# dkales/dpf-go

Hardware: AMD Instinct MI355X
Metric: DPF leaf points/sec (EvalFull logN=20, batched keys) + AES blocks/sec (higher is better)
Workload: dtype u32

## Files before the change

dpf-go_amd/csrc/dpf_capi.hip:

```cpp
#include <hip/hip_runtime.h>
#include <sched.h>
#include <stdint.h>
#include <stdio.h>
#include <stdlib.h>
#include <string.h>
#include <sys/mman.h>

#include <algorithm>
#include <atomic>
#include <condition_variable>
#include <functional>
#include <memory>
#include <mutex>
#include <unordered_map>
#include <string>
#include <thread>
#include <vector>

#include "../../include/dpf_hip.h"
#include "dpf_internal.hpp"
#include "bs_kernels.hpp"
#include "dpf_kernels.hpp"
#include "pir_kernels.hpp"

// ... 324 lines not shown
}

bool want_bs() { return g_aes_impl.load(std::memory_order_relaxed) == DPF_AES_BITSLICED; }

hipError_t expand_keys(const uint8_t* d_keys, size_t klen, size_t nk, uint32_t stop, const TreeWs& w, hipStream_t st,
                       bool bs) {
    if (bs) return dpfk::launch_unpack_both(d_keys, klen, nk, stop, w.ek, w.ekb, st);
    return dpfk::launch_unpack(d_keys, klen, nk, stop, w.ek, st);
}

hipError_t run_tree(const TreeWs& w, size_t k0, size_t n, uint32_t stop, uint32_t prefix_bits, uint64_t prefix,
                    uint8_t* out, uint64_t stride, hipStream_t st, bool bs) {
    if (bs && dpfk::bs_applicable(stop, prefix_bits))
        return dpfk::launch_evalfull_bs(w.ek + k0 * dpfk::ek_words(stop), w.ekb + k0 * dpfk::bs_key_words(stop), n, stop,
                                        prefix_bits, prefix, out, stride, w.frontier, st);
    return dpfk::launch_evalfull(w.ek + k0 * dpfk::ek_words(stop), n, stop, prefix_bits, prefix, out, stride, st);
}

hipError_t tree_from_keys(const uint8_t* d_keys, size_t klen, size_t nk, uint32_t stop, uint32_t prefix_bits,
                          uint64_t prefix, uint8_t* out, uint64_t stride, void* d_work, hipStream_t st, bool bs,
                          bool* expanded) {
    if (!bs && dpfk::evalfull_raw_ok(nk, stop, prefix_bits)) {
        *expanded = false;
        return dpfk::launch_evalfull_raw(d_keys, klen, nk, stop, prefix_bits, prefix, out, stride, st);
    }
    *expanded = true;
    const TreeWs w = tree_ws(d_work, nk, stop);
    hipError_t e = expand_keys(d_keys, klen, nk, stop, w, st, bs);
    return e != hipSuccess ? e : run_tree(w, 0, nk, stop, prefix_bits, prefix, out, stride, st, bs);
}

constexpr size_t kStageBytes = (size_t)32 << 20;
constexpr size_t kSlabMinOut = (size_t)8 << 20;

int ensure_staging(Dev& d, size_t chunk_cap) {
    if (!d.cst) {
        HIP_TRY(hipStreamCreateWithFlags(&d.cst, hipStreamNonBlocking));
        for (int i = 0; i < 2; ++i) {
            HIP_TRY(hipEventCreateWithFlags(&d.ev_k[i], hipEventDisableTiming));
// ... 61 lines not shown
    HIP_TRY(hipMemcpyAsync(d.keys.p, keys, nk * klen, hipMemcpyHostToDevice, d.st));
    const TreeWs w = tree_ws(d.work.p, nk, stop);
    const bool bs = want_bs();
    const uint8_t* dk = (const uint8_t*)d.keys.p;
    uint32_t pb = 0;
    while ((olen >> pb) > kStageBytes) ++pb;
    if (olen >= kSlabMinOut && pb < 2) pb = 2;
    const bool raw = !bs && (pb == 0 ? dpfk::evalfull_raw_ok(std::min(per, nk), stop, 0) &&
                                                       (nk % per == 0 || dpfk::evalfull_raw_ok(nk % per, stop, 0))
                                                 : dpfk::evalfull_raw_ok(1, stop, pb));
    if (!raw) HIP_TRY(expand_keys(dk, klen, nk, stop, w, d.st, bs));
    if (pb == 0) {
        const size_t nch = (nk + per - 1) / per;
        return pipeline_d2h(d, nch, std::min(per, nk) * olen, [&](size_t i, uint8_t* dbuf, size_t& bytes, size_t& off) {
            const size_t k0 = i * per, n = std::min(per, nk - k0);
            if (raw) HIP_TRY(dpfk::launch_evalfull_raw(dk + k0 * klen, klen, n, stop, 0, 0, dbuf, olen, d.st));
            else HIP_TRY(run_tree(w, k0, n, stop, 0, 0, dbuf, olen, d.st, bs));
            bytes = n * olen;
            off = k0 * olen;
            return DPF_OK;
        }, out, nk * olen);
    }
    const size_t slab = olen >> pb, per_key = (size_t)1 << pb;
    return pipeline_d2h(d, nk * per_key, slab, [&](size_t i, uint8_t* dbuf, size_t& bytes, size_t& off) {
        const size_t k = i / per_key, p = i % per_key;
        if (raw) HIP_TRY(dpfk::launch_evalfull_raw(dk + k * klen, klen, 1, stop, pb, p, dbuf, slab, d.st));
        else HIP_TRY(run_tree(w, k, 1, stop, pb, p, dbuf, slab, d.st, bs));
        bytes = slab;
        off = k * olen + p * slab;
        return DPF_OK;
    }, out, nk * olen);
}

size_t pir_ek_bytes(size_t nkeys, uint32_t logN);
size_t eval_work_bytes(size_t nkeys, size_t ppk, uint32_t logN);

int eval_on_device(Dev& d, const uint8_t* keys, size_t klen, size_t nk, const uint64_t* xs, size_t ppk,
                   uint32_t logN, uint8_t* out) {
    std::lock_guard<std::mutex> lk(d.mu);
    DeviceGuard g(d.id);
    const uint32_t stop = stop_of(logN);
// ... 298 lines not shown
        std::lock_guard<std::mutex> lk(d.mu);
        DeviceGuard gd(d.id);
        HIP_TRY(hipError_t(d.keys.ensure(klen)));
        HIP_TRY(hipError_t(d.work.ensure(tree_ws_bytes(1, stop, pb, 1))));
        HIP_TRY(hipMemcpyAsync(d.keys.p, key, klen, hipMemcpyHostToDevice, d.st));
        const TreeWs w = tree_ws(d.work.p, 1, stop);
        const bool bs = want_bs();
        const uint8_t* dk = (const uint8_t*)d.keys.p;
        uint32_t extra = 0;
        while ((slab >> extra) > kStageBytes && pb + extra < stop) ++extra;
        const size_t sub = slab >> extra;
        const bool raw = !bs && dpfk::evalfull_raw_ok(1, stop, pb + extra);
        if (!raw) HIP_TRY(expand_keys(dk, klen, 1, stop, w, d.st, bs));
        return pipeline_d2h(d, (size_t)1 << extra, sub, [&](size_t j, uint8_t* dbuf, size_t& bytes, size_t& off) {
            const uint64_t p = ((uint64_t)lo << extra) + j;
            if (raw) HIP_TRY(dpfk::launch_evalfull_raw(dk, klen, 1, stop, pb + extra, p, dbuf, sub, d.st));
            else HIP_TRY(run_tree(w, 0, 1, stop, pb + extra, p, dbuf, sub, d.st, bs));
            bytes = sub;
            off = lo * slab + j * sub;
            return DPF_OK;
        }, out + lo * slab, slab, lo * slab);
    });
}

int dpf_evalfull_subtree_dev(int device, const uint8_t* d_keys, size_t klen, size_t nkeys, uint32_t logN,
                             uint32_t prefix_bits, uint64_t prefix, uint8_t* d_out, void* d_work, void* stream) {
    if (int rc = check_key(klen, logN)) return rc;
    const uint32_t stop = stop_of(logN);
    if (prefix_bits > stop || (prefix_bits < 64 && (prefix >> prefix_bits) != 0))
        return fail(DPF_ERR_PARAM, "dpf: subtree prefix out of range");
    if (nkeys == 0) return DPF_OK;
    DeviceGuard g(device);
    CuScope cus(stream);
    const bool bs = want_bs();
    bool expanded = false;
    forget_expanded(d_work);
    HIP_TRY(tree_from_keys(d_keys, klen, nkeys, stop, prefix_bits, prefix, d_out, (uint64_t)16 << (stop - prefix_bits),
                           d_work, (hipStream_t)stream, bs, &expanded));
    if (expanded) note_expanded(d_work, nkeys, stop, bs);
    return DPF_OK;
}

int dpf_evalfull_batch_dev(int device, const uint8_t* d_keys, size_t klen, size_t nkeys, uint32_t logN,
                           uint8_t* d_out, void* d_work, void* stream) {
    return dpf_evalfull_subtree_dev(device, d_keys, klen, nkeys, logN, 0, 0, d_out, d_work, stream);
}

size_t dpf_eval_workspace_size(size_t nkeys, size_t pts_per_key, uint32_t logN) {
    return std::max<size_t>(16, eval_work_bytes(nkeys, pts_per_key, logN));
}

uint32_t dpf_eval_frontier_level(uint32_t logN, size_t pts_per_key) {
    return logN > 63 ? 0 : dpfk::eval_frontier_level(stop_of(logN), pts_per_key);
}
// ... 417 lines not shown
```

dpf-go_amd/csrc/dpf_kernels.hip:

```cpp
#include <hip/hip_runtime.h>
#include <stdint.h>
#include <stdlib.h>

#include <algorithm>
#include <atomic>
#include <cmath>
#include <mutex>
#include <type_traits>
#include "aes_consts.hpp"
#include "aes_ttable.hpp"
#include "dpf_kernels.hpp"
#include "wave_prio.hpp"
#include "tree_ops.hpp"

namespace dpfk {

#ifdef DPF_WAVE_TIMES
constexpr uint64_t kWaveTimesMax = 1u << 16;
__device__ uint64_t g_wave_times[5 * kWaveTimesMax];
#endif

struct Ctx {
    const uint8_t* tab;
    uint32_t lo;
    KeySrc ks;
    Blk fcw;
    uint8_t* outp;
    uint4* nseed;
    uint8_t* nt;
    uint32_t groups;
    uint32_t* prog = nullptr;
    uint32_t pslot = 0;
};

// ... 55 lines not shown
        ob = leaf_fix(ob, b.t, c.fcw);
        o2 = oa;
        o3 = ob;
        if (h == 0) {
            o0 = oa;
            o1 = ob;
        }
        m = pend;
    }
    store16(p, o0);
    store16(p + 16, o1);
    store16(p + 32, o2);
    store16(p + 48, o3);
}

template <int DMAX, int D, bool NODES, bool PAIR, bool B, bool RAW = false>
__device__ __forceinline__ void dfs(Ctx& c, uint32_t lvl0, const Node& n) {
    if constexpr (PAIR && D == 3) {
        CW cw = key_cw<RAW>(c.ks, lvl0 + DMAX - 3);
        Node L, R;
        expand<B>(c.tab, c.lo, n, cw, L, R);
        const bool odd = (threadIdx.x & 1u) != 0;
        const Node got = pair_swap(sel(odd, L, R));
        const int64_t sub = 16ll << DMAX;
        Node cur = sel(odd, got, L);
        const Node second = sel(odd, R, got);
#pragma nounroll
        for (int h = 0; h < 2; ++h) {
            leaves4<B, RAW>(c, lvl0 + DMAX - 2, cur, c.outp + (h == 0 ? (odd ? 64 - sub : 0) : (odd ? 64 : sub)));
            prio_step<DMAX>(c);
            cur = second;
        }
        c.outp += 128;
    } else if constexpr (D == 0) {
        if constexpr (NODES) {
            emit_node(c, n);
        } else {
            Blk o = mmo1(c.tab, c.lo, KeyFixed<false>{}, n.s);
            store16(c.outp, leaf_fix(o, n.t, c.fcw));
            c.outp += 16;
        }
    } else if constexpr (D == 2 && !NODES) {
        leaves4<B, RAW>(c, lvl0 + DMAX - 2, n, c.outp);
// ... 24 lines not shown
        } else {
            Blk oL, oR;
            mmo2<B>(c.tab, c.lo, KeyFixed<false>{}, L.s, oL, KeyFixed<false>{}, R.s, oR);
            store16(c.outp, leaf_fix(oL, L.t, c.fcw));
            store16(c.outp + 16, leaf_fix(oR, R.t, c.fcw));
            c.outp += 32;
        }
    } else {
        CW cw = key_cw<RAW>(c.ks, lvl0 + DMAX - D);
        Node L, R;
        expand<B>(c.tab, c.lo, n, cw, L, R);
        Node ch = L;
        const Node pend = R;
#pragma nounroll
        for (int side = 0; side < 2; ++side) {
            dfs<DMAX, D - 1, NODES, PAIR, B, RAW>(c, lvl0, ch);
            ch = pend;
        }
    }
}

__global__ void k_unpack(const uint8_t* __restrict__ keys, uint64_t key_len, uint64_t nkeys, uint32_t stop,
                         uint32_t* __restrict__ ek) {
    const uint64_t recs = (uint64_t)stop + 2;
    const uint64_t i = (uint64_t)blockIdx.x * blockDim.x + threadIdx.x;
    if (i >= nkeys * recs) return;
    const uint64_t k = i / recs, r = i % recs;
    const uint8_t* kp = keys + k * key_len;
    uint32_t* o = ek + k * (recs * 8) + r * 8;
    auto w = [](const uint8_t* p) {
        return (uint32_t)p[0] | ((uint32_t)p[1] << 8) | ((uint32_t)p[2] << 16) | ((uint32_t)p[3] << 24);
    };
    if (r == 0) {
        o[0] = w(kp); o[1] = w(kp + 4); o[2] = w(kp + 8); o[3] = w(kp + 12);
        o[4] = kp[16]; o[5] = 0; o[6] = 0; o[7] = 0;
    } else if (r <= stop) {
        const uint8_t* p = kp + 17 + 18 * (r - 1);
        o[0] = w(p); o[1] = w(p + 4); o[2] = w(p + 8); o[3] = w(p + 12);
        o[4] = p[16]; o[5] = p[17]; o[6] = 0; o[7] = 0;
    } else {
        const uint8_t* p = kp + key_len - 16;
        o[0] = w(p); o[1] = w(p + 4); o[2] = w(p + 8); o[3] = w(p + 12);
        o[4] = 0; o[5] = 0; o[6] = 0; o[7] = 0;
    }
}

template <int D, bool UNIFORM, bool NODES, bool RAW = false>
__global__ __launch_bounds__(kTreeBlockMax, kTreeWaves) void k_evalfull(const uint32_t* __restrict__ ekeys, uint32_t stop,
                                                        uint64_t nunits, uint32_t units_log, uint32_t ltop,
                                                        uint64_t sub_base, uint8_t* __restrict__ out,
                                                        uint8_t* __restrict__ out_t, uint64_t out_stride,
                                                        uint64_t klen = 0, uint64_t kboff = 0) {
    static_assert(!RAW || (UNIFORM && !NODES), "raw keys: wave-uniform leaf launches only");
#ifdef DPF_WAVE_TIMES
    const uint64_t t_start = wall_clock64();
#endif
    __shared__ __attribute__((aligned(16))) uint32_t s_tab[kTabWords];
    const uint32_t B = blockDim.x, W = 31u - (uint32_t)__builtin_clz(B);
    const uint64_t u = (uint64_t)blockIdx.x * B + threadIdx.x;
    uint64_t key = u >> units_log;
    if constexpr (UNIFORM) key = __builtin_amdgcn_readfirstlane((uint32_t)key);
    const uint64_t local = u & ((1ull << units_log) - 1);
    const uint64_t sub = sub_base + local;
    Ctx c;
    if constexpr (RAW) {
        c.ks = {nullptr, ekeys, kboff + key * klen, klen};
    } else {
        c.ks = {ekeys + key * ((uint64_t)(stop + 2) * 8), nullptr, 0, 0};
// ... 80 lines not shown
            n = get(threadIdx.x >> (W - F));
            lvl = l1;
        }
    }
    if (cw_lds) {
        for (uint32_t i = lvl; i < ltop; ++i)
            walk_step<true>(c.tab, c.lo, n, lds_cw(i), (uint32_t)(sub >> (ltop - 1 - i)) & 1u);
    } else {
        for (uint32_t i = lvl; i < ltop; ++i)
            walk_step<true>(c.tab, c.lo, n, key_cw<RAW>(c.ks, i), (uint32_t)(sub >> (ltop - 1 - i)) & 1u);
    }
#ifdef DPF_WAVE_TIMES
    const uint64_t t_walk = wall_clock64();
#endif
    constexpr bool kPair = UNIFORM && !NODES && D >= 3;
    dfs<D, D, NODES, kPair, UNIFORM, RAW>(c, ltop, n);
    if (c.prog != nullptr) c.prog[c.pslot] = 0xffffffffu;
#ifdef DPF_WAVE_TIMES
    if ((threadIdx.x & 63) == 0) {
        const uint64_t wv = u >> 6;
        if (wv < kWaveTimesMax) {
            g_wave_times[5 * wv] = t_start;
            g_wave_times[5 * wv + 1] = wall_clock64();
            g_wave_times[5 * wv + 2] = __builtin_amdgcn_s_getreg(0xF804);
            g_wave_times[5 * wv + 3] = __builtin_amdgcn_s_getreg(0xF814);
            g_wave_times[5 * wv + 4] = t_walk;
        }
    }
#endif
}

__device__ __forceinline__ Node eval_start(const uint32_t* ek, uint64_t key, uint64_t x, uint32_t logN,
                                           const uint4* fseed, const uint8_t* ft, uint32_t L) {
    Node n;
    if (fseed != nullptr) {
        const uint64_t idx = (key << L) + ((x >> (logN - L)) & ((1ull << L) - 1));
        const uint4 v = fseed[idx];
        n.s = {v.x, v.y, v.z, v.w};
        n.t = ft[idx];
    } else {
        n.s = load_blk(ek);
// ... 437 lines not shown
    while (b < maxb && n > cus * b) b <<= 1;
    return b;
}

struct TreeShape {
    uint32_t d, block;
};
static TreeShape pick_shape(uint32_t span, uint64_t nkeys, bool nodes, uint32_t prefix_bits) {
    static const int forced = [] {
        const char* e = getenv("DPF_SUBTREE_DEPTH");
        return e ? atoi(e) : -1;
    }();
    const uint32_t dmax = span < kMaxD ? span : kMaxD;
    auto threads = [&](uint32_t dd) { return span - dd >= 40 ? ~0ull : nkeys << (span - dd); };
    auto block = [&](uint32_t dd) {
        return pick_block(threads(dd), !nodes && dd >= kBigMinD ? (uint32_t)kTreeBlockBig : (uint32_t)kTreeBlock);
    };
    if (forced >= 0) {
        const uint32_t d = dmax < (uint32_t)forced ? dmax : (uint32_t)forced;
        return {d, block(d)};
    }
    constexpr double kLat = 1.9e-6;
    constexpr double kPerWave = 0.2e-6;
    const double wave_slots = 64.0 * cu_count();
    uint32_t best = dmax;
    double best_t = 1e30;
    for (int dd = (int)dmax; dd >= 0; --dd) {
        const uint32_t d = (uint32_t)dd;
        double walk = (double)(span - d), lat = 0.0;
        const double w = (double)threads(d) / wave_slots;
        const double rounds = w > 16.0 ? std::ceil(w / 16.0) : 1.0;
// ... 34 lines not shown
}
template <class F>
static void with_depth(uint32_t d, F&& f) {
    switch (d) {
        case 0: return f(std::integral_constant<int, 0>{});
        case 1: return f(std::integral_constant<int, 1>{});
        case 2: return f(std::integral_constant<int, 2>{});
        case 3: return f(std::integral_constant<int, 3>{});
        case 4: return f(std::integral_constant<int, 4>{});
        case 5: return f(std::integral_constant<int, 5>{});
        case 6: return f(std::integral_constant<int, 6>{});
        default: return f(std::integral_constant<int, 7>{});
    }
}

template <bool NODES>
static hipError_t launch_tree(const uint32_t* ek, uint64_t nkeys, uint32_t stop, uint32_t depth,
                              uint32_t prefix_bits, uint64_t prefix, uint8_t* out, uint8_t* out_t,
                              uint64_t out_stride, hipStream_t st) {
    const TreeLaunch t = tree_launch(nkeys, depth, prefix_bits, prefix, NODES);
    if (t.nunits == 0) return hipSuccess;
    with_depth(t.d, [&](auto dd) {
        constexpr int D = decltype(dd)::value;
        if (t.units_log >= 6)
            hipLaunchKernelGGL((k_evalfull<D, true, NODES>), t.grid, t.block, 0, st, ek, stop, t.nunits, t.units_log,
                               t.ltop, t.sub_base, out, out_t, out_stride);
        else
            hipLaunchKernelGGL((k_evalfull<D, false, NODES>), t.grid, t.block, 0, st, ek, stop, t.nunits, t.units_log,
                               t.ltop, t.sub_base, out, out_t, out_stride);
    });
    return hipGetLastError();
}

bool evalfull_raw_ok(uint64_t nkeys, uint32_t stop, uint32_t prefix_bits) {
    static const bool on = [] {
        const char* e = getenv("DPF_RAW_KEYS");
        return !(e && e[0] == '0');
    }();
    if (!on || nkeys == 0 || prefix_bits > stop) return false;
    return tree_launch(nkeys, stop, prefix_bits, 0, false).units_log >= 6;
}

hipError_t launch_evalfull_raw(const uint8_t* keys, uint64_t klen, uint64_t nkeys, uint32_t stop, uint32_t prefix_bits,
                               uint64_t prefix, uint8_t* out, uint64_t out_stride, hipStream_t st) {
    const TreeLaunch t = tree_launch(nkeys, stop, prefix_bits, prefix, false);
    if (t.units_log < 6) return hipErrorInvalidValue;
    const uint64_t kboff = (uintptr_t)keys & 3;
    const uint32_t* kw = reinterpret_cast<const uint32_t*>(keys - kboff);
    with_depth(t.d, [&](auto dd) {
        hipLaunchKernelGGL((k_evalfull<decltype(dd)::value, true, false, true>), t.grid, t.block, 0, st, kw, stop,
                           t.nunits, t.units_log, t.ltop, t.sub_base, out, nullptr, out_stride, klen, kboff);
    });
    return hipGetLastError();
}

hipError_t launch_nodes(const uint32_t* ek, uint64_t nkeys, uint32_t stop, uint32_t depth, uint32_t prefix_bits,
                        uint64_t prefix, uint8_t* seeds, uint8_t* ts, uint64_t stride, hipStream_t st) {
    return launch_tree<true>(ek, nkeys, stop, depth, prefix_bits, prefix, seeds, ts, stride, st);
}

hipError_t launch_evalfull(const uint32_t* ek, uint64_t nkeys, uint32_t stop, uint32_t prefix_bits,
                           uint64_t prefix, uint8_t* out, uint64_t out_stride, hipStream_t st) {
    return launch_tree<false>(ek, nkeys, stop, stop, prefix_bits, prefix, out, nullptr, out_stride, st);
}

uint32_t eval_frontier_level(uint32_t stop, uint64_t pts_per_key) {
    uint32_t L = 0;
    while (L < kMaxFrontierHbm && L < stop && (2ull << (L + 1)) <= pts_per_key) ++L;
    static const int shift = [] {
        const char* e = getenv("DPF_EVAL_LEVEL_SHIFT");
        return e && *e ? atoi(e) : 0;
    }();
    if (L >= 4 && shift > 0 && L + (uint32_t)shift < stop && L + (uint32_t)shift <= kMaxFrontierHbm) L += shift;
    return L >= 4 ? L : 0;
}

uint64_t eval_frontier_bytes(uint64_t nkeys, uint32_t stop, uint64_t pts_per_key) {
    const uint32_t L = eval_frontier_level(stop, pts_per_key);
// ... 95 lines not shown
```

dpf-go_amd/csrc/dpf_kernels.hpp:

```cpp
#pragma once
#include <hip/hip_runtime.h>
#include <stdint.h>

namespace dpfk {

constexpr int kBlock = 512;
constexpr int kTreeBlock = 512;
constexpr int kTreeBlockBig = 1024;
constexpr int kTreeBlockMax = 1024;
constexpr uint32_t kBigMinD = 6;
constexpr uint32_t kFeedbackMinD = 6;
constexpr int kTreeWaves = 4;
constexpr uint32_t kMaxD = 7;
constexpr uint32_t kMaxFrontierHbm = 16;

void set_cu_budget(int cus);
int cu_budget();
int cu_count();

inline uint64_t ek_words(uint32_t stop) { return ((uint64_t)stop + 2) * 8; }

hipError_t launch_mmo_tt(const uint8_t* in, uint8_t* out, uint64_t nblocks, uint32_t right, uint32_t reps,
                         hipStream_t st);

hipError_t launch_unpack(const uint8_t* keys, uint64_t key_len, uint64_t nkeys, uint32_t stop, uint32_t* ek,
                         hipStream_t st);

hipError_t launch_evalfull(const uint32_t* ek, uint64_t nkeys, uint32_t stop, uint32_t prefix_bits,
                           uint64_t prefix, uint8_t* out, uint64_t out_stride, hipStream_t st);

bool evalfull_raw_ok(uint64_t nkeys, uint32_t stop, uint32_t prefix_bits);
hipError_t launch_evalfull_raw(const uint8_t* keys, uint64_t klen, uint64_t nkeys, uint32_t stop, uint32_t prefix_bits,
                               uint64_t prefix, uint8_t* out, uint64_t out_stride, hipStream_t st);

hipError_t launch_nodes(const uint32_t* ek, uint64_t nkeys, uint32_t stop, uint32_t depth, uint32_t prefix_bits,
                        uint64_t prefix, uint8_t* seeds, uint8_t* ts, uint64_t stride, hipStream_t st);

uint32_t eval_frontier_level(uint32_t stop, uint64_t pts_per_key);
int set_eval_trie(int on);
int get_eval_trie();
bool eval_trie_built();
uint64_t eval_frontier_bytes(uint64_t nkeys, uint32_t stop, uint64_t pts_per_key);
hipError_t launch_eval(const uint32_t* ek, uint32_t stop, uint32_t logN, const uint64_t* xs, uint64_t nq,
                       uint64_t pts_per_key, uint8_t* out, void* frontier, uint64_t frontier_bytes,
                       hipStream_t st);

}
```

dpf-go_amd/dpf/__init__.py:

```python
from __future__ import annotations

import ctypes
import os
from typing import Optional, Sequence, Tuple

import numpy as np

_HERE = os.path.dirname(os.path.abspath(__file__))
LIB_PATH = os.environ.get("DPF_LIB") or os.path.join(os.path.dirname(_HERE), "lib", "libdpf_hip.so")
HEADER_PATH = os.path.join(os.path.dirname(os.path.dirname(_HERE)), "include", "dpf_hip.h")

DPF_OK = 0
DPF_ERR_PARAM = -1
DPF_ERR_KEYLEN = -2
DPF_ERR_NODEV = -3
DPF_ERR_HIP = -4
DPF_ERR_NOMEM = -5
AES_TTABLE = 0
AES_BITSLICED = 1


class DPFPanic(RuntimeError):

    def __init__(self, code: int, msg: str):
# ... 18 lines not shown
    "dpf_gpu_init_devices": (_int, [ctypes.POINTER(_int), _int]),
    "dpf_gpu_shutdown": (None, []),
    "dpf_gpu_count": (_int, []),
    "dpf_gen_seeded": (_int, [_u64, _u32, _u8p, _u8p, _u8p, _u8p]),
    "dpf_gen": (_int, [_u64, _u32, _u8p, _u8p]),
    "dpf_gen_batch_seeded": (_int, [_u64p, _u32, _u8p, _u8p, _sz, _u8p, _u8p, _int]),
    "dpf_keys_pack": (_int, [ctypes.POINTER(_vp), ctypes.POINTER(_sz), _sz, _sz, _u8p]),
    "dpf_keys_unpack": (_int, [_u8p, _sz, _sz, ctypes.POINTER(_vp)]),
    "dpf_eval": (_int, [_u8p, _sz, _u64, _u32, _u8p]),
    "dpf_evalfull": (_int, [_u8p, _sz, _u32, _u8p]),
    "dpf_evalfull_batch": (_int, [_u8p, _sz, _sz, _u32, _u8p, _int]),
    "dpf_eval_batch": (_int, [_u8p, _sz, _sz, _u64p, _sz, _u32, _u8p, _int]),
    "dpf_evalfull_split": (_int, [_u8p, _sz, _u32, _u8p, _int]),
    "dpf_evalfull_batch_dev": (_int, [_int, _vp, _sz, _sz, _u32, _vp, _vp, _vp]),
    "dpf_evalfull_subtree_dev": (_int, [_int, _vp, _sz, _sz, _u32, _u32, _u64, _vp, _vp, _vp]),
    "dpf_eval_workspace_size": (_sz, [_sz, _sz, _u32]),
    "dpf_eval_frontier_level": (_u32, [_u32, _sz]),
    "dpf_eval_batch_dev": (_int, [_int, _vp, _sz, _sz, _vp, _sz, _u32, _vp, _vp, _sz, _vp]),
    "dpf_expand_keys_dev": (_int, [_int, _vp, _sz, _sz, _u32, _vp, _vp]),
    "dpf_evalfull_expanded_dev": (_int, [_int, _vp, _sz, _u32, _u32, _u64, _vp, _vp]),
    "dpf_forget_workspace": (_int, [_vp]),
    "dpf_set_small_call_path": (_int, [_int]),
    "dpf_get_small_call_path": (_int, []),
    "dpf_small_call_max_logN": (ctypes.c_uint32, []),
    "dpf_set_aes_impl": (_int, [_int]),
    "dpf_get_aes_impl": (_int, []),
    "dpf_set_eval_kernel": (_int, [_int]),
    "dpf_get_eval_kernel": (_int, []),
    "dpf_set_pir_kernel": (_int, [_int]),
    "dpf_get_pir_kernel": (_int, []),
# ... 59 lines not shown
    return np.frombuffer(bytes(b), dtype=np.uint8)


def key_len(logN: int) -> int:
    return int(lib().dpf_key_len(logN))


def evalfull_len(logN: int) -> int:
    return int(lib().dpf_evalfull_len(logN))


def workspace_size(nkeys: int, logN: int) -> int:
    return int(lib().dpf_workspace_size(nkeys, logN))


def gpu_init(ngpus: int = 0) -> int:
    rc = lib().dpf_gpu_init(ngpus)
    if rc < 0:
        _check(rc)
    return rc


def gpu_init_devices(ordinals: Sequence[int]) -> int:
    ids = (_int * len(ordinals))(*ordinals)
    rc = lib().dpf_gpu_init_devices(ids, len(ordinals))
    if rc < 0:
        _check(rc)
    return rc


# ... 371 lines not shown
```

include/dpf_hip.h:

```cpp
#ifndef DPF_HIP_H
#define DPF_HIP_H

#include <stddef.h>
#include <stdint.h>

#ifdef __cplusplus
extern "C" {
#endif

#define DPF_OK 0
#define DPF_ERR_PARAM (-1)
#define DPF_ERR_KEYLEN (-2)
#define DPF_ERR_NODEV (-3)
#define DPF_ERR_HIP (-4)
#define DPF_ERR_NOMEM (-5)

const char* dpf_last_error(void);

size_t dpf_key_len(uint32_t logN);
size_t dpf_evalfull_len(uint32_t logN);
size_t dpf_workspace_size(size_t nkeys, uint32_t logN);

int dpf_gpu_init(int ngpus);
int dpf_gpu_init_devices(const int* ordinals, int n);
// ... 6 lines not shown
int dpf_gen_batch_seeded(const uint64_t* alphas, uint32_t logN, const uint8_t* s0s, const uint8_t* s1s, size_t n,
                         uint8_t* kas, uint8_t* kbs, int nthreads);

int dpf_keys_pack(const uint8_t* const* keys, const size_t* lens, size_t n, size_t key_len, uint8_t* out);
int dpf_keys_unpack(const uint8_t* packed, size_t key_len, size_t n, uint8_t* const* keys);

int dpf_eval(const uint8_t* key, size_t key_len, uint64_t x, uint32_t logN, uint8_t* out_bit);
int dpf_evalfull(const uint8_t* key, size_t key_len, uint32_t logN, uint8_t* out);
int dpf_evalfull_batch(const uint8_t* keys, size_t key_len, size_t nkeys, uint32_t logN, uint8_t* out, int ngpus);
int dpf_eval_batch(const uint8_t* keys, size_t key_len, size_t nkeys, const uint64_t* xs, size_t pts_per_key,
                   uint32_t logN, uint8_t* out, int ngpus);
int dpf_evalfull_split(const uint8_t* key, size_t key_len, uint32_t logN, uint8_t* out, int ngpus);

int dpf_evalfull_batch_dev(int device, const uint8_t* d_keys, size_t key_len, size_t nkeys, uint32_t logN,
                           uint8_t* d_out, void* d_work, void* stream);
int dpf_evalfull_subtree_dev(int device, const uint8_t* d_keys, size_t key_len, size_t nkeys, uint32_t logN,
                             uint32_t prefix_bits, uint64_t prefix, uint8_t* d_out, void* d_work, void* stream);
size_t dpf_eval_workspace_size(size_t nkeys, size_t pts_per_key, uint32_t logN);
uint32_t dpf_eval_frontier_level(uint32_t logN, size_t pts_per_key);
int dpf_eval_batch_dev(int device, const uint8_t* d_keys, size_t key_len, size_t nkeys, const uint64_t* d_xs,
                       size_t pts_per_key, uint32_t logN, uint8_t* d_out, void* d_work, size_t work_bytes,
                       void* stream);

int dpf_stream_create_cu_masked(int device, uint32_t cu_first, uint32_t cu_count, void** stream);
int dpf_stream_destroy(void* stream);

#define DPF_AES_TTABLE 0
#define DPF_AES_BITSLICED 1
int dpf_set_aes_impl(int impl);
int dpf_get_aes_impl(void);
// ... 70 lines not shown
```

Measured before the change: 4618 billion.

## Add inter-wave work stealing for deep EvalFull leaf subtrees and tune block choice

Adds an optional work-stealing scheme to the tree evaluation kernel. Each wave expands its subtree frontier into a shared workspace and publishes progress. Idle waves scan for unfinished jobs and claim trailing units through atomics, to even out tail imbalance. Stealing is off by default behind an environment variable. The launch heuristic is also changed to choose between big and small blocks by comparing idle CUs against extra blocks, which can change occupancy for mid-sized launches.

```diff
diff --git a/dpf-go_amd/csrc/dpf_capi.hip b/dpf-go_amd/csrc/dpf_capi.hip
--- a/dpf-go_amd/csrc/dpf_capi.hip
+++ b/dpf-go_amd/csrc/dpf_capi.hip
@@ -362,7 +362,8 @@
     if (bs && dpfk::bs_applicable(stop, prefix_bits))
         return dpfk::launch_evalfull_bs(w.ek + k0 * dpfk::ek_words(stop), w.ekb + k0 * dpfk::bs_key_words(stop), n, stop,
                                         prefix_bits, prefix, out, stride, w.frontier, st);
-    return dpfk::launch_evalfull(w.ek + k0 * dpfk::ek_words(stop), n, stop, prefix_bits, prefix, out, stride, st);
+    return dpfk::launch_evalfull(w.ek + k0 * dpfk::ek_words(stop), n, stop, prefix_bits, prefix, out, stride, st,
+                                 w.frontier);
 }
 
 hipError_t tree_from_keys(const uint8_t* d_keys, size_t klen, size_t nk, uint32_t stop, uint32_t prefix_bits,
@@ -370,7 +371,8 @@
                           bool* expanded) {
     if (!bs && dpfk::evalfull_raw_ok(nk, stop, prefix_bits)) {
         *expanded = false;
-        return dpfk::launch_evalfull_raw(d_keys, klen, nk, stop, prefix_bits, prefix, out, stride, st);
+        return dpfk::launch_evalfull_raw(d_keys, klen, nk, stop, prefix_bits, prefix, out, stride, st,
+                                         d_work != nullptr ? tree_ws(d_work, nk, stop).frontier : nullptr);
     }
     *expanded = true;
     const TreeWs w = tree_ws(d_work, nk, stop);
@@ -462,7 +464,7 @@
         const size_t nch = (nk + per - 1) / per;
         return pipeline_d2h(d, nch, std::min(per, nk) * olen, [&](size_t i, uint8_t* dbuf, size_t& bytes, size_t& off) {
             const size_t k0 = i * per, n = std::min(per, nk - k0);
-            if (raw) HIP_TRY(dpfk::launch_evalfull_raw(dk + k0 * klen, klen, n, stop, 0, 0, dbuf, olen, d.st));
+            if (raw) HIP_TRY(dpfk::launch_evalfull_raw(dk + k0 * klen, klen, n, stop, 0, 0, dbuf, olen, d.st, w.frontier));
             else HIP_TRY(run_tree(w, k0, n, stop, 0, 0, dbuf, olen, d.st, bs));
             bytes = n * olen;
             off = k0 * olen;
@@ -472,7 +474,7 @@
     const size_t slab = olen >> pb, per_key = (size_t)1 << pb;
     return pipeline_d2h(d, nk * per_key, slab, [&](size_t i, uint8_t* dbuf, size_t& bytes, size_t& off) {
         const size_t k = i / per_key, p = i % per_key;
-        if (raw) HIP_TRY(dpfk::launch_evalfull_raw(dk + k * klen, klen, 1, stop, pb, p, dbuf, slab, d.st));
+        if (raw) HIP_TRY(dpfk::launch_evalfull_raw(dk + k * klen, klen, 1, stop, pb, p, dbuf, slab, d.st, w.frontier));
         else HIP_TRY(run_tree(w, k, 1, stop, pb, p, dbuf, slab, d.st, bs));
         bytes = slab;
         off = k * olen + p * slab;
@@ -801,7 +803,7 @@
         if (!raw) HIP_TRY(expand_keys(dk, klen, 1, stop, w, d.st, bs));
         return pipeline_d2h(d, (size_t)1 << extra, sub, [&](size_t j, uint8_t* dbuf, size_t& bytes, size_t& off) {
             const uint64_t p = ((uint64_t)lo << extra) + j;
-            if (raw) HIP_TRY(dpfk::launch_evalfull_raw(dk, klen, 1, stop, pb + extra, p, dbuf, sub, d.st));
+            if (raw) HIP_TRY(dpfk::launch_evalfull_raw(dk, klen, 1, stop, pb + extra, p, dbuf, sub, d.st, w.frontier));
             else HIP_TRY(run_tree(w, 0, 1, stop, pb + extra, p, dbuf, sub, d.st, bs));
             bytes = sub;
             off = lo * slab + j * sub;
@@ -825,6 +827,13 @@
     HIP_TRY(tree_from_keys(d_keys, klen, nkeys, stop, prefix_bits, prefix, d_out, (uint64_t)16 << (stop - prefix_bits),
                            d_work, (hipStream_t)stream, bs, &expanded));
     if (expanded) note_expanded(d_work, nkeys, stop, bs);
+    return DPF_OK;
+}
+
+int dpf_tree_steal_stats(int device, uint64_t* stolen, uint64_t* run_twice) {
+    if (stolen == nullptr || run_twice == nullptr) return fail(DPF_ERR_PARAM, "dpf: null statistics pointer");
+    DeviceGuard g(device);
+    HIP_TRY(dpfk::steal_last_stats(stolen, run_twice));
     return DPF_OK;
 }
 
diff --git a/dpf-go_amd/csrc/dpf_kernels.hip b/dpf-go_amd/csrc/dpf_kernels.hip
--- a/dpf-go_amd/csrc/dpf_kernels.hip
+++ b/dpf-go_amd/csrc/dpf_kernels.hip
@@ -7,17 +7,20 @@
 #include <cmath>
 #include <mutex>
 #include <type_traits>
+#include <vector>
 #include "aes_consts.hpp"
 #include "aes_ttable.hpp"
 #include "dpf_kernels.hpp"
 #include "wave_prio.hpp"
 #include "tree_ops.hpp"
+#include "tree_steal.hpp"
 
 namespace dpfk {
 
 #ifdef DPF_WAVE_TIMES
 constexpr uint64_t kWaveTimesMax = 1u << 16;
-__device__ uint64_t g_wave_times[5 * kWaveTimesMax];
+constexpr int kWaveTimesCols = 7;
+__device__ uint64_t g_wave_times[kWaveTimesCols * kWaveTimesMax];
 #endif
 
 struct Ctx {
@@ -103,19 +106,23 @@
     store16(p + 48, o3);
 }
 
-template <int DMAX, int D, bool NODES, bool PAIR, bool B, bool RAW = false>
-__device__ __forceinline__ void dfs(Ctx& c, uint32_t lvl0, const Node& n) {
+struct NoHook {
+    __device__ __forceinline__ void operator()() const {}
+};
+template <int DMAX, int D, bool NODES, bool PAIR, bool B, bool RAW = false, int SUBLOG = DMAX, class Hook = NoHook>
+__device__ __forceinline__ void dfs(Ctx& c, uint32_t lvl0, const Node& n, const Hook& hook = Hook{}) {
     if constexpr (PAIR && D == 3) {
         CW cw = key_cw<RAW>(c.ks, lvl0 + DMAX - 3);
         Node L, R;
         expand<B>(c.tab, c.lo, n, cw, L, R);
         const bool odd = (threadIdx.x & 1u) != 0;
         const Node got = pair_swap(sel(odd, L, R));
-        const int64_t sub = 16ll << DMAX;
+        const int64_t sub = 16ll << SUBLOG;
         Node cur = sel(odd, got, L);
         const Node second = sel(odd, R, got);
 #pragma nounroll
         for (int h = 0; h < 2; ++h) {
+            if (h == 1) hook();
             leaves4<B, RAW>(c, lvl0 + DMAX - 2, cur, c.outp + (h == 0 ? (odd ? 64 - sub : 0) : (odd ? 64 : sub)));
             prio_step<DMAX>(c);
             cur = second;
@@ -170,10 +177,171 @@
         const Node pend = R;
 #pragma nounroll
         for (int side = 0; side < 2; ++side) {
-            dfs<DMAX, D - 1, NODES, PAIR, B, RAW>(c, lvl0, ch);
+            dfs<DMAX, D - 1, NODES, PAIR, B, RAW, SUBLOG>(c, lvl0, ch);
             ch = pend;
         }
     }
+}
+
+struct StealOps {
+    static __device__ __forceinline__ uint32_t load(const uint32_t& w) {
+        return __hip_atomic_load(&w, __ATOMIC_RELAXED, __HIP_MEMORY_SCOPE_AGENT);
+    }
+    static __device__ __forceinline__ void store(uint32_t& w, uint32_t v) {
+        __hip_atomic_store(&w, v, __ATOMIC_RELAXED, __HIP_MEMORY_SCOPE_AGENT);
+    }
+    static __device__ __forceinline__ uint32_t fetch_add(uint32_t& w, uint32_t v) {
+        return __hip_atomic_fetch_add(&w, v, __ATOMIC_RELAXED, __HIP_MEMORY_SCOPE_AGENT);
+    }
+    static __device__ __forceinline__ void release() { __builtin_amdgcn_fence(__ATOMIC_RELEASE, "agent"); }
+    static __device__ __forceinline__ void acquire() { __builtin_amdgcn_fence(__ATOMIC_ACQUIRE, "agent"); }
+};
+
+template <int K, bool RAW>
+__device__ __forceinline__ void steal_front(const Ctx& c, uint32_t lvl, const Node& n, uint4*& fs, uint32_t& tw,
+                                            uint32_t& i) {
+    if constexpr (K == 0) {
+        *fs = make_uint4(n.s.c0, n.s.c1, n.s.c2, n.s.c3);
+        fs += 64;
+        tw |= (n.t != 0 ? 1u : 0u) << i;
+        ++i;
+    } else {
+        CW cw = key_cw<RAW>(c.ks, lvl);
+        Node L, R;
+        expand<true>(c.tab, c.lo, n, cw, L, R);
+        Node ch = L;
+        const Node pend = R;
+#pragma nounroll
+        for (int side = 0; side < 2; ++side) {
+            steal_front<K - 1, RAW>(c, lvl + 1, ch, fs, tw, i);
+            ch = pend;
+        }
+    }
+}
+
+constexpr uint32_t kStealScanSlices = 4;
+constexpr uint32_t kStealScan = 64 * kStealScanSlices;
+
+template <int D, bool RAW>
+__device__ __forceinline__ uint32_t steal_stages(Ctx& c, const StealArgs& sa, const uint32_t* ekeys, uint32_t stop,
+                                                 uint64_t nunits, uint32_t units_log, uint32_t ltop, uint8_t* out,
+                                                 uint64_t out_stride, uint64_t klen, uint64_t kboff, uint64_t u0,
+                                                 const Node& root, uint64_t& t_front) {
+    constexpr int K = D - 3;
+    constexpr uint32_t U = 1u << K;
+    using Job = StealJob<uint32_t>;
+    Job* const jobs = reinterpret_cast<Job*>(sa.state);
+    const uint32_t lane = threadIdx.x & 63u;
+    const uint32_t njobs = (uint32_t)(nunits >> 6);
+    const uint32_t myjob = __builtin_amdgcn_readfirstlane((uint32_t)(u0 >> 6));
+    {
+        uint4* fs = sa.fseed + (((uint64_t)myjob * 64) << K) + lane;
+        uint32_t tw = 0, i = 0;
+        steal_front<K, RAW>(c, ltop, root, fs, tw, i);
+        sa.ft[(uint64_t)myjob * 64 + lane] = tw;
+    }
+    steal_publish<StealOps>(jobs[myjob]);
+    __builtin_amdgcn_fence(__ATOMIC_ACQUIRE, "workgroup");
+#ifdef DPF_WAVE_TIMES
+    t_front = wall_clock64();
+#else
+    (void)t_front;
+#endif
+    struct Raw {
+        uint4 v;
+        uint32_t w;
+    };
+    auto load_node = [&](uint32_t j, uint32_t unit) __attribute__((always_inline)) {
+        return Raw{sa.fseed[(((uint64_t)j * 64) << K) + unit * 64 + lane], sa.ft[(uint64_t)j * 64 + lane]};
+    };
+    auto node_of = [&](const Raw& r, uint32_t unit) __attribute__((always_inline)) {
+        return Node{{r.v.x, r.v.y, r.v.z, r.v.w}, (r.w >> unit) & 1u};
+    };
+    uint32_t job = myjob, unit = 0, stolen = 0, seen = 0, misses = 0;
+    uint32_t win = (myjob + 16u) % njobs;
+    bool own = true;
+    Raw nx = load_node(job, 0);
+    Node cur = node_of(nx, 0);
+    const bool skewed = sa.skew != 0 && (myjob & 1u) != 0;
+    auto ahead = [&]() __attribute__((always_inline)) {
+        if (own) {
+            seen = steal_owner_begin<StealOps>(jobs[job], unit, U);
+            if (unit + 1 < U) nx = load_node(job, unit + 1);
+        }
+    };
+    for (;;) {
+        if (own && skewed)
+            for (uint32_t i = 0; i < sa.skew; ++i) __builtin_amdgcn_s_sleep(127);
+        {
+            const uint64_t ju = (uint64_t)job * 64;
+            const uint64_t key = ju >> units_log, local = (ju & ((1ull << units_log) - 1)) + lane;
+            c.outp = out + key * out_stride + local * (16ull << D) + unit * 128u;
+        }
+        dfs<D, 3, false, true, true, RAW, D>(c, ltop, cur, ahead);
+        if (own) {
+            if (steal_owner_next(unit, U, __builtin_amdgcn_readfirstlane(seen))) {
+                ++unit;
+                cur = node_of(nx, unit);
+                continue;
+            }
+            steal_owner_done<StealOps>(jobs[job], unit + 1);
+            own = false;
+        }
+        bool got = false;
+        while (!got && misses * kStealScan < njobs + kStealScan) {
+            uint32_t best = 0, bestj = 0;
+#pragma unroll
+            for (uint32_t s = 0; s < kStealScanSlices; ++s) {
+                const uint32_t o = s * 64 + lane;
+                const uint32_t j = win + o < njobs ? win + o : win + o - njobs;
+                if (o < njobs) {
+                    const uint32_t a = steal_avail(StealOps::load(jobs[j].prog), StealOps::load(jobs[j].thieves), U);
+                    const uint32_t k = a == 0 || j == myjob ? 0u : (a << 8) | ((j * 37u + myjob) & 0xffu);
+                    if (k > best) {
+                        best = k;
+                        bestj = j;
+                    }
+                }
+            }
+            uint32_t m = best;
+#pragma unroll
+            for (int sh = 1; sh < 64; sh <<= 1) m = max(m, (uint32_t)__shfl_xor((int)m, sh));
+            m = __builtin_amdgcn_readfirstlane(m);
+            if (m == 0) {
+                ++misses;
+                win = win + kStealScan < njobs ? win + kStealScan : (win + kStealScan) % njobs;
+                continue;
+            }
+            const uint64_t who = __ballot(best == m);
+            const uint32_t wl = (uint32_t)__builtin_ctzll(who);
+            const uint32_t j = (uint32_t)__builtin_amdgcn_readlane((int)bestj, (int)wl);
+            uint32_t cu = 0, ok = 0;
+            if (lane == 0) ok = steal_claim<StealOps>(jobs[j], U, cu) && steal_claim_needed<StealOps>(jobs[j], cu) ? 1u : 0u;
+            ok = __builtin_amdgcn_readfirstlane(ok);
+            cu = __builtin_amdgcn_readfirstlane(cu);
+            if (ok == 0) {
+                ++misses;
+                continue;
+            }
+            steal_acquire<StealOps>();
+            got = true;
+            job = j;
+            unit = cu;
+            ++stolen;
+        }
+        if (!got) break;
+        {
+            const uint64_t key = ((uint64_t)job * 64) >> units_log;
+            if constexpr (RAW) {
+                c.ks = {nullptr, ekeys, kboff + key * klen, klen};
+            } else {
+                c.ks = {ekeys + key * ((uint64_t)(stop + 2) * 8), nullptr, 0, 0};
+            }
+            c.fcw = key_fcw<RAW>(c.ks, stop);
+        }
+        cur = node_of(load_node(job, unit), unit);
+    }
+    return stolen;
 }
 
 __global__ void k_unpack(const uint8_t* __restrict__ keys, uint64_t key_len, uint64_t nkeys, uint32_t stop,
@@ -201,13 +369,15 @@
     }
 }
 
-template <int D, bool UNIFORM, bool NODES, bool RAW = false>
+template <int D, bool UNIFORM, bool NODES, bool RAW = false, bool STEAL = false>
 __global__ __launch_bounds__(kTreeBlockMax, kTreeWaves) void k_evalfull(const uint32_t* __restrict__ ekeys, uint32_t stop,
                                                         uint64_t nunits, uint32_t units_log, uint32_t ltop,
                                                         uint64_t sub_base, uint8_t* __restrict__ out,
                                                         uint8_t* __restrict__ out_t, uint64_t out_stride,
-                                                        uint64_t klen = 0, uint64_t kboff = 0) {
+                                                        uint64_t klen = 0, uint64_t kboff = 0,
+                                                        StealArgs sa = StealArgs{}) {
     static_assert(!RAW || (UNIFORM && !NODES), "raw keys: wave-uniform leaf launches only");
+    static_assert(!STEAL || (UNIFORM && !NODES && D >= (int)kBigMinD), "STEAL: wave-uniform deep leaf launches only");
 #ifdef DPF_WAVE_TIMES
     const uint64_t t_start = wall_clock64();
 #endif
@@ -318,17 +488,27 @@
     const uint64_t t_walk = wall_clock64();
 #endif
     constexpr bool kPair = UNIFORM && !NODES && D >= 3;
-    dfs<D, D, NODES, kPair, UNIFORM, RAW>(c, ltop, n);
+    [[maybe_unused]] uint64_t t_front = 0;
+    [[maybe_unused]] uint32_t stolen = 0;
+    if constexpr (STEAL) {
+        stolen = steal_stages<D, RAW>(c, sa, ekeys, stop, nunits, units_log, ltop, out, out_stride, klen, kboff, u, n,
+                                      t_front);
+    } else {
+        dfs<D, D, NODES, kPair, UNIFORM, RAW>(c, ltop, n);
+    }
     if (c.prog != nullptr) c.prog[c.pslot] = 0xffffffffu;
 #ifdef DPF_WAVE_TIMES
     if ((threadIdx.x & 63) == 0) {
         const uint64_t wv = u >> 6;
         if (wv < kWaveTimesMax) {
-            g_wave_times[5 * wv] = t_start;
-            g_wave_times[5 * wv + 1] = wall_clock64();
-            g_wave_times[5 * wv + 2] = __builtin_amdgcn_s_getreg(0xF804);
-            g_wave_times[5 * wv + 3] = __builtin_amdgcn_s_getreg(0xF814);
-            g_wave_times[5 * wv + 4] = t_walk;
+            uint64_t* const r = g_wave_times + kWaveTimesCols * wv;
+            r[0] = t_start;
+            r[1] = wall_clock64();
+            r[2] = __builtin_amdgcn_s_getreg(0xF804);
+            r[3] = __builtin_amdgcn_s_getreg(0xF814);
+            r[4] = t_walk;
+            r[5] = STEAL ? t_front : t_walk;
+            r[6] = stolen;
         }
     }
 #endif
@@ -796,7 +976,14 @@
     const uint32_t dmax = span < kMaxD ? span : kMaxD;
     auto threads = [&](uint32_t dd) { return span - dd >= 40 ? ~0ull : nkeys << (span - dd); };
     auto block = [&](uint32_t dd) {
-        return pick_block(threads(dd), !nodes && dd >= kBigMinD ? (uint32_t)kTreeBlockBig : (uint32_t)kTreeBlock);
+        const uint64_t n = threads(dd), cus = (uint64_t)cu_count();
+        bool big = !nodes && dd >= kBigMinD;
+        if (big && n < cus * kTreeBlockBig && n > cus * kTreeBlock) {
+            const uint64_t idle = cus - (n + kTreeBlockBig - 1) / kTreeBlockBig;
+            const uint64_t dbl = (n + kTreeBlock - 1) / kTreeBlock - cus;
+            big = dbl >= idle;
+        }
+        return pick_block(n, big ? (uint32_t)kTreeBlockBig : (uint32_t)kTreeBlock);
     };
     if (forced >= 0) {
         const uint32_t d = dmax < (uint32_t)forced ? dmax : (uint32_t)forced;
@@ -861,12 +1048,89 @@
     }
 }
 
+static bool steal_on() {
+    static const bool on = [] {
+        const char* e = getenv("DPF_TREE_STEAL");
+        return e && *e ? e[0] != '0' : kStealDefault;
+    }();
+    return on;
+}
+static uint32_t steal_skew() {
+    static const uint32_t k = [] {
+        const char* e = getenv("DPF_TREE_STEAL_SKEW");
+        const int v = e && *e ? atoi(e) : 0;
+        return (uint32_t)(v < 0 ? 0 : v > 4096 ? 4096 : v);
+    }();
+    return k;
+}
+uint64_t steal_ws_bytes(uint64_t nkeys, uint32_t stop, uint32_t prefix_bits) {
+    if (stop < prefix_bits + kBigMinD + 6) return 0;
+    const uint64_t n = nkeys << (stop - 3 - prefix_bits);
+    return (n * 16 + n + 255) & ~255ull;
+}
+static bool steal_applies(const TreeLaunch& t, const void* ws) {
+    const uint64_t njobs = t.nunits >> 6;
+    return ws != nullptr && steal_on() && t.d >= kBigMinD && t.units_log >= 6 && njobs >= 2 &&
+           t.nunits <= (uint64_t)cu_count() * kTreeBlockBig;
+}
+struct StealLast {
+    const void* state = nullptr;
+    uint32_t njobs = 0, units = 0;
+};
+static std::mutex g_steal_mu;
+static StealLast g_steal_last[64];
+static hipError_t steal_prepare(const TreeLaunch& t, void* ws, hipStream_t st, StealArgs& sa) {
+    const uint32_t njobs = (uint32_t)(t.nunits >> 6);
+    uint8_t* p = static_cast<uint8_t*>(ws);
+    sa.fseed = reinterpret_cast<uint4*>(p);
+    sa.ft = reinterpret_cast<uint32_t*>(p + ((t.nunits << (t.d - 3)) * 16));
+    sa.state = sa.ft + t.nunits;
+    sa.skew = steal_skew();
+    int dev = 0;
+    if (hipGetDevice(&dev) == hipSuccess && dev >= 0 && dev < 64) {
+        std::lock_guard<std::mutex> lk(g_steal_mu);
+        g_steal_last[dev] = {sa.state, njobs, 1u << (t.d - 3)};
+    }
+    return hipMemsetAsync(sa.state, 0, (size_t)njobs * kStealStateWords * 4, st);
+}
+hipError_t steal_last_stats(uint64_t* stolen, uint64_t* twice) {
+    *stolen = *twice = 0;
+    int dev = 0;
+    hipError_t e = hipGetDevice(&dev);
+    if (e != hipSuccess) return e;
+    StealLast l;
+    if (dev >= 0 && dev < 64) {
+        std::lock_guard<std::mutex> lk(g_steal_mu);
+        l = g_steal_last[dev];
+    }
+    if ((e = hipDeviceSynchronize()) != hipSuccess) return e;
+    if (l.state == nullptr) return hipSuccess;
+    std::vector<uint32_t> w((size_t)l.njobs * kStealStateWords);
+    if ((e = hipMemcpy(w.data(), l.state, w.size() * 4, hipMemcpyDeviceToHost)) != hipSuccess) return e;
+    for (uint32_t j = 0; j < l.njobs; ++j) steal_stats(w[4 * j + 1], w[4 * j + 2], w[4 * j + 3], l.units, *stolen, *twice);
+    return hipSuccess;
+}
+
 template <bool NODES>
 static hipError_t launch_tree(const uint32_t* ek, uint64_t nkeys, uint32_t stop, uint32_t depth,
                               uint32_t prefix_bits, uint64_t prefix, uint8_t* out, uint8_t* out_t,
-                              uint64_t out_stride, hipStream_t st) {
+                              uint64_t out_stride, hipStream_t st, void* steal_ws = nullptr) {
     const TreeLaunch t = tree_launch(nkeys, depth, prefix_bits, prefix, NODES);
     if (t.nunits == 0) return hipSuccess;
+    if constexpr (!NODES) {
+        if (steal_applies(t, steal_ws)) {
+            StealArgs sa;
+            hipError_t e = steal_prepare(t, steal_ws, st, sa);
+            if (e != hipSuccess) return e;
+            if (t.d == 6)
+                hipLaunchKernelGGL((k_evalfull<6, true, false, false, true>), t.grid, t.block, 0, st, ek, stop, t.nunits,
+                                   t.units_log, t.ltop, t.sub_base, out, out_t, out_stride, 0ull, 0ull, sa);
+            else
+                hipLaunchKernelGGL((k_evalfull<7, true, false, false, true>), t.grid, t.block, 0, st, ek, stop, t.nunits,
+                                   t.units_log, t.ltop, t.sub_base, out, out_t, out_stride, 0ull, 0ull, sa);
+            return hipGetLastError();
+        }
+    }
     with_depth(t.d, [&](auto dd) {
         constexpr int D = decltype(dd)::value;
         if (t.units_log >= 6)
@@ -889,11 +1153,23 @@
 }
 
 hipError_t launch_evalfull_raw(const uint8_t* keys, uint64_t klen, uint64_t nkeys, uint32_t stop, uint32_t prefix_bits,
-                               uint64_t prefix, uint8_t* out, uint64_t out_stride, hipStream_t st) {
+                               uint64_t prefix, uint8_t* out, uint64_t out_stride, hipStream_t st, void* steal_ws) {
     const TreeLaunch t = tree_launch(nkeys, stop, prefix_bits, prefix, false);
     if (t.units_log < 6) return hipErrorInvalidValue;
     const uint64_t kboff = (uintptr_t)keys & 3;
     const uint32_t* kw = reinterpret_cast<const uint32_t*>(keys - kboff);
+    if (steal_applies(t, steal_ws)) {
+        StealArgs sa;
+        hipError_t e = steal_prepare(t, steal_ws, st, sa);
+        if (e != hipSuccess) return e;
+        if (t.d == 6)
+            hipLaunchKernelGGL((k_evalfull<6, true, false, true, true>), t.grid, t.block, 0, st, kw, stop, t.nunits,
+                               t.units_log, t.ltop, t.sub_base, out, nullptr, out_stride, klen, kboff, sa);
+        else
+            hipLaunchKernelGGL((k_evalfull<7, true, false, true, true>), t.grid, t.block, 0, st, kw, stop, t.nunits,
+                               t.units_log, t.ltop, t.sub_base, out, nullptr, out_stride, klen, kboff, sa);
+        return hipGetLastError();
+    }
     with_depth(t.d, [&](auto dd) {
         hipLaunchKernelGGL((k_evalfull<decltype(dd)::value, true, false, true>), t.grid, t.block, 0, st, kw, stop,
                            t.nunits, t.units_log, t.ltop, t.sub_base, out, nullptr, out_stride, klen, kboff);
@@ -907,8 +1183,8 @@
 }
 
 hipError_t launch_evalfull(const uint32_t* ek, uint64_t nkeys, uint32_t stop, uint32_t prefix_bits,
-                           uint64_t prefix, uint8_t* out, uint64_t out_stride, hipStream_t st) {
-    return launch_tree<false>(ek, nkeys, stop, stop, prefix_bits, prefix, out, nullptr, out_stride, st);
+                           uint64_t prefix, uint8_t* out, uint64_t out_stride, hipStream_t st, void* steal_ws) {
+    return launch_tree<false>(ek, nkeys, stop, stop, prefix_bits, prefix, out, nullptr, out_stride, st, steal_ws);
 }
 
 uint32_t eval_frontier_level(uint32_t stop, uint64_t pts_per_key) {
diff --git a/dpf-go_amd/csrc/dpf_kernels.hpp b/dpf-go_amd/csrc/dpf_kernels.hpp
--- a/dpf-go_amd/csrc/dpf_kernels.hpp
+++ b/dpf-go_amd/csrc/dpf_kernels.hpp
@@ -1,6 +1,7 @@
 #pragma once
 #include <hip/hip_runtime.h>
 #include <stdint.h>
+#include "tree_steal.hpp"
 
 namespace dpfk {
 
@@ -27,11 +28,23 @@
                          hipStream_t st);
 
 hipError_t launch_evalfull(const uint32_t* ek, uint64_t nkeys, uint32_t stop, uint32_t prefix_bits,
-                           uint64_t prefix, uint8_t* out, uint64_t out_stride, hipStream_t st);
+                           uint64_t prefix, uint8_t* out, uint64_t out_stride, hipStream_t st,
+                           void* steal_ws = nullptr);
+
+constexpr bool kStealDefault = false;
+struct StealArgs {
+    uint4* fseed = nullptr;
+    uint32_t* ft = nullptr;
+    uint32_t* state = nullptr;
+    uint32_t skew = 0;
+};
+uint64_t steal_ws_bytes(uint64_t nkeys, uint32_t stop, uint32_t prefix_bits);
+hipError_t steal_last_stats(uint64_t* stolen, uint64_t* twice);
 
 bool evalfull_raw_ok(uint64_t nkeys, uint32_t stop, uint32_t prefix_bits);
 hipError_t launch_evalfull_raw(const uint8_t* keys, uint64_t klen, uint64_t nkeys, uint32_t stop, uint32_t prefix_bits,
-                               uint64_t prefix, uint8_t* out, uint64_t out_stride, hipStream_t st);
+                               uint64_t prefix, uint8_t* out, uint64_t out_stride, hipStream_t st,
+                               void* steal_ws = nullptr);
 
 hipError_t launch_nodes(const uint32_t* ek, uint64_t nkeys, uint32_t stop, uint32_t depth, uint32_t prefix_bits,
                         uint64_t prefix, uint8_t* seeds, uint8_t* ts, uint64_t stride, hipStream_t st);
diff --git a/dpf-go_amd/csrc/tree_steal.hpp b/dpf-go_amd/csrc/tree_steal.hpp
--- /dev/null
+++ b/dpf-go_amd/csrc/tree_steal.hpp
@@ -0,0 +1,76 @@
+#pragma once
+#include <stdint.h>
+
+#if defined(__HIP__) || defined(__HIPCC__)
+#define DPF_STEAL_FN __host__ __device__ __forceinline__
+#else
+#define DPF_STEAL_FN inline
+#endif
+
+namespace dpfk {
+
+constexpr uint32_t kStealReady = 0x80000000u;
+constexpr uint32_t kStealProgMask = 0xffffu;
+constexpr uint32_t kStealStateWords = 4;
+
+template <class W>
+struct StealJob {
+    W prog, thieves, ran, waived;
+};
+
+template <class Ops, class W>
+DPF_STEAL_FN void steal_publish(StealJob<W>& j) {
+    Ops::release();
+    Ops::store(j.prog, kStealReady | 1u);
+}
+
+template <class Ops, class W>
+DPF_STEAL_FN uint32_t steal_owner_begin(StealJob<W>& j, uint32_t u, uint32_t U) {
+    const uint32_t c = u + 2 < U ? u + 2 : U;
+    Ops::store(j.prog, kStealReady | c);
+    return Ops::load(j.thieves);
+}
+
+DPF_STEAL_FN bool steal_owner_next(uint32_t u, uint32_t U, uint32_t thieves_seen) {
+    const uint32_t t = thieves_seen < U ? thieves_seen : U;
+    return u + 1 < U - t;
+}
+
+template <class Ops, class W>
+DPF_STEAL_FN void steal_owner_done(StealJob<W>& j, uint32_t ran) {
+    Ops::store(j.ran, ran);
+}
+
+DPF_STEAL_FN uint32_t steal_avail(uint32_t prog, uint32_t thieves, uint32_t U) {
+    if ((prog & kStealReady) == 0) return 0;
+    const uint32_t used = (prog & kStealProgMask) + thieves;
+    return used < U ? U - used : 0;
+}
+
+template <class Ops, class W>
+DPF_STEAL_FN bool steal_claim(StealJob<W>& j, uint32_t U, uint32_t& unit, uint32_t* t_old = nullptr) {
+    const uint32_t t = Ops::fetch_add(j.thieves, 1u);
+    if (t_old != nullptr) *t_old = t;
+    if (t >= U) return false;
+    unit = U - 1 - t;
+    return true;
+}
+template <class Ops, class W>
+DPF_STEAL_FN bool steal_claim_needed(StealJob<W>& j, uint32_t unit) {
+    if ((Ops::load(j.prog) & kStealProgMask) < unit + 2) return true;
+    Ops::fetch_add(j.waived, 1u);
+    return false;
+}
+template <class Ops>
+DPF_STEAL_FN void steal_acquire() {
+    Ops::acquire();
+}
+
+inline void steal_stats(uint32_t thieves, uint32_t ran, uint32_t waived, uint32_t U, uint64_t& stolen,
+                        uint64_t& twice) {
+    const uint32_t t = (thieves < U ? thieves : U) - waived;
+    stolen += t;
+    if (ran + t > U) twice += ran + t - U;
+}
+
+}
diff --git a/dpf-go_amd/dpf/__init__.py b/dpf-go_amd/dpf/__init__.py
--- a/dpf-go_amd/dpf/__init__.py
+++ b/dpf-go_amd/dpf/__init__.py
@@ -56,6 +56,7 @@
     "dpf_evalfull_split": (_int, [_u8p, _sz, _u32, _u8p, _int]),
     "dpf_evalfull_batch_dev": (_int, [_int, _vp, _sz, _sz, _u32, _vp, _vp, _vp]),
     "dpf_evalfull_subtree_dev": (_int, [_int, _vp, _sz, _sz, _u32, _u32, _u64, _vp, _vp, _vp]),
+    "dpf_tree_steal_stats": (_int, [_int, _u64p, _u64p]),
     "dpf_eval_workspace_size": (_sz, [_sz, _sz, _u32]),
     "dpf_eval_frontier_level": (_u32, [_u32, _sz]),
     "dpf_eval_batch_dev": (_int, [_int, _vp, _sz, _sz, _vp, _sz, _u32, _vp, _vp, _sz, _vp]),
@@ -145,6 +146,12 @@
     return int(lib().dpf_workspace_size(nkeys, logN))
 
 
+def tree_steal_stats(device: int = 0) -> tuple:
+    st, tw = ctypes.c_uint64(0), ctypes.c_uint64(0)
+    _check(lib().dpf_tree_steal_stats(device, ctypes.byref(st), ctypes.byref(tw)))
+    return int(st.value), int(tw.value)
+
+
 def gpu_init(ngpus: int = 0) -> int:
     rc = lib().dpf_gpu_init(ngpus)
     if rc < 0:
diff --git a/include/dpf_hip.h b/include/dpf_hip.h
--- a/include/dpf_hip.h
+++ b/include/dpf_hip.h
@@ -44,6 +44,7 @@
 
 int dpf_evalfull_batch_dev(int device, const uint8_t* d_keys, size_t key_len, size_t nkeys, uint32_t logN,
                            uint8_t* d_out, void* d_work, void* stream);
+int dpf_tree_steal_stats(int device, uint64_t* stolen, uint64_t* run_twice);
 int dpf_evalfull_subtree_dev(int device, const uint8_t* d_keys, size_t key_len, size_t nkeys, uint32_t logN,
                              uint32_t prefix_bits, uint64_t prefix, uint8_t* d_out, void* d_work, void* stream);
 size_t dpf_eval_workspace_size(size_t nkeys, size_t pts_per_key, uint32_t logN);
```

Result: no change. 4617 billion, median of 2 (-0.0%).
